# kubernetes-sigs/scheduler-plugins

Measured on AMD Instinct MI355X. Metric: pod_x_node_filter_score_evals_per_sec, higher is better.
Workload: dtype f32+f64

## Files before the change

### include/spx.h

```cpp
#ifndef SPX_H
#define SPX_H

#include <stdint.h>

#ifdef __cplusplus
extern "C" {
#endif


#define SPX_OK 0
#define SPX_ERR_ARG (-1)
#define SPX_ERR_HIP (-2)
#define SPX_ERR_STATE (-3)
#define SPX_ERR_NOGPU (-4)

#define SPX_PLUGIN_ALLOCATABLE 0
#define SPX_PLUGIN_TLP 1
#define SPX_PLUGIN_LVRB 2
#define SPX_PLUGIN_NRT 3
#define SPX_PLUGIN_NETOVERHEAD 4
#define SPX_PLUGIN_CAPACITY 5
#define SPX_PLUGIN_TOPOSORT 6
#define SPX_PLUGIN_LROC 7
#define SPX_PLUGIN_PEAKS 8
// ... 714 lines not shown
#define SPX_OPT_PEAKS_POD_CLASSES 8
#define SPX_OPT_NRT_LN_LIST_PERMILLE 9
#define SPX_OPT_COMMIT_COOP 10
#define SPX_OPT_NRT_RANK_FILTER 11
#define SPX_OPT_ROW_WORKGROUP 12
#define SPX_OPT_TLP_AMB_TABLE 13
#define SPX_OPT_NRT_PACKED_SCORE 14
#define SPX_OPT_NET_ALLOC_FUSED 15
#define SPX_OPT_NRT_RANK_NARROW 16
#define SPX_OPT_PEAKS_ESTIMATE 17
#define SPX_OPT_NRT_FUSED 18
#define SPX_OPT_NRT_WIDE 19
#define SPX_OPT_ALLOC_TABLE_KEEP 20
#define SPX_OPT_TLP_POD_CLASSES 21
#define SPX_OPT_TLP_CHUNK_SCHED 22
#define SPX_NUM_OPTIONS 23
int spx_set_option(spx_engine* e, int option, int64_t value);
int spx_get_option(const spx_engine* e, int option, int64_t* value);

int spx_nrt_pod_classes(const spx_engine* e, int64_t* n_unique, int64_t* n_copies);
int spx_peaks_pod_classes(const spx_engine* e, int64_t* n_unique, int64_t* n_copies);

int spx_tlp_pod_classes(const spx_engine* e, int64_t* rows_evaluated, int64_t* rows_copied);
int spx_tlp_form(const spx_engine* e);
int spx_tlp_fetch_order(spx_engine* e, int32_t* rows);

int spx_sysched_pod_classes(const spx_engine* e, int64_t* n_unique, int64_t* n_copies);

int spx_load_trimaran(spx_engine* e, const spx_node_objects* nodes, const spx_resource_classes* rc, const spx_pod_objects* pods, const spx_metrics_objects* metrics, const spx_assigned_objects* assigned);
int spx_load_trimaran_pods(spx_engine* e, const spx_pod_objects* pods);
int spx_load_nrt(spx_engine* e, const spx_node_objects* nodes, const spx_nrt_objects* nrt, const spx_resource_classes* rc, const spx_pod_objects* pods, const spx_nrt_params* params);
int spx_last_load_nrt_ms(const spx_engine* e, double* ms6);
int spx_load_network(spx_engine* e, const spx_node_objects* nodes, const spx_pod_objects* pods, const spx_appgroup_objects* appgroups, const spx_nettopo_objects* nettopo);
int spx_load_quota(spx_engine* e, const spx_pod_objects* pods, const spx_resource_classes* rc, const spx_quota_objects* quota);
int spx_load_sysched(spx_engine* e, const spx_sysched_objects* o);
typedef struct spx_profile_objects {
  const spx_node_objects* nodes;
  const spx_resource_classes* rc;
  const spx_pod_objects* pods;
// ... 131 lines not shown
```

### scheduler-plugins_amd/csrc/kernels_tlp_order.hip

```cpp
#include <hip/hip_runtime.h>

#include "spx_internal.h"

namespace spx {
namespace {

constexpr int kBlock = 1024;
constexpr int kSlots = 2 * kBlock;
constexpr uint32_t kEmpty = 0xffffffffu;

__device__ __forceinline__ uint32_t order_bin(int64_t v, int32_t amb_size) {
  return (v >= 0 && v < static_cast<int64_t>(amb_size)) ? static_cast<uint32_t>(v) : static_cast<uint32_t>(amb_size);
}

__device__ __forceinline__ void block_count(uint32_t* skey, uint32_t* scnt, bool live, uint32_t bin, uint32_t* slot, uint32_t* rank) {
  for (int s = threadIdx.x; s < kSlots; s += kBlock) skey[s] = kEmpty, scnt[s] = 0u;
  __syncthreads();
  *slot = 0u, *rank = 0u;
  if (live) {
    uint32_t s = (bin * 2654435761u) >> 21;
    for (;;) {
      const uint32_t prev = atomicCAS(skey + s, kEmpty, bin);
      if (prev == kEmpty || prev == bin) break;
      s = (s + 1u) & (kSlots - 1);
// ... 15 lines not shown
    if (skey[s] != kEmpty) atomicAdd(hist + skey[s], scnt[s]);
}

__device__ __forceinline__ uint32_t block_sum(uint32_t v, uint32_t* wsum) {
#pragma unroll
  for (int m = 32; m >= 1; m >>= 1) v += static_cast<uint32_t>(__shfl_xor(static_cast<int>(v), m));
  if ((threadIdx.x & 63) == 0) wsum[threadIdx.x >> 6] = v;
  __syncthreads();
  uint32_t total = 0;
#pragma unroll
  for (int w = 0; w < kBlock / 64; ++w) total += wsum[w];
  __syncthreads();
  return total;
}

__global__ __launch_bounds__(kBlock) void k_tlp_order_totals(const uint32_t* hist, int n_bins, uint32_t* totals) {
  __shared__ uint32_t wsum[kBlock / 64];
  const int b = blockIdx.x * kBlock + threadIdx.x;
  const uint32_t total = block_sum(b < n_bins ? hist[b] : 0u, wsum);
  if (threadIdx.x == 0) totals[blockIdx.x] = total;
}

__global__ __launch_bounds__(kBlock) void k_tlp_order_scan(uint32_t* hist, int n_bins, const uint32_t* totals, uint32_t* other_start, uint32_t* evaluated) {
  __shared__ uint32_t wsum[kBlock / 64];
  const int t = threadIdx.x, lane = t & 63, wave = t >> 6;
  uint32_t mine = 0;
  for (int i = t; i < static_cast<int>(blockIdx.x); i += kBlock) mine += totals[i];
  const uint32_t carry = block_sum(mine, wsum);
  const int b = blockIdx.x * kBlock + t;
  const uint32_t c = b < n_bins ? hist[b] : 0u;
  uint32_t x = c;
#pragma unroll
  for (int d = 1; d < 64; d <<= 1) {
    const uint32_t y = static_cast<uint32_t>(__shfl_up(static_cast<int>(x), d));
    if (lane >= d) x += y;
  }
  if (lane == 63) wsum[wave] = x;
  __syncthreads();
  uint32_t before = 0;
#pragma unroll
  for (int w = 0; w < kBlock / 64; ++w) before += w < wave ? wsum[w] : 0u;
  __syncthreads();
  const uint32_t o = carry + before + x - c;
  uint32_t ev = 0;
  if (b < n_bins) {
    hist[b] = o;
    if (b == n_bins - 1) *other_start = o;
    else if (c > 0u) ev = 1u + ((o + c - 1u) >> 6) - (o >> 6);
  }
  ev = block_sum(ev, wsum);
  if (t == 0 && ev != 0u) atomicAdd(evaluated, ev);
}

__global__ __launch_bounds__(kBlock) void k_tlp_order_scatter(const int64_t* pod, int64_t n, int32_t amb_size, uint32_t* cursor, int32_t* order) {
  __shared__ uint32_t skey[kSlots], scnt[kSlots];
  const int64_t r = static_cast<int64_t>(blockIdx.x) * kBlock + threadIdx.x;
  const bool live = r < n;
  uint32_t slot, rank;
  block_count(skey, scnt, live, live ? order_bin(pod[r], amb_size) : 0u, &slot, &rank);
  for (int s = threadIdx.x; s < kSlots; s += kBlock)
    if (skey[s] != kEmpty) scnt[s] = atomicAdd(cursor + skey[s], scnt[s]);
  __syncthreads();
  if (live) {
    const uint64_t pos = static_cast<uint64_t>(scnt[slot]) + rank;
    if (pos < static_cast<uint64_t>(n)) order[pos] = static_cast<int32_t>(r);
  }
}

__global__ __launch_bounds__(256) void k_tlp_order_count_key(const int64_t* pod, int64_t n, int32_t amb_size, const int32_t* order, const uint32_t* other_start,
                                                             uint32_t* evaluated, uint32_t* keys, int64_t n_chunks) {
  const int64_t p = static_cast<int64_t>(blockIdx.x) * blockDim.x + threadIdx.x;
  const uint32_t last = static_cast<uint32_t>(n - 1);
  bool ev = false, outside = false;
  if (p < n) {
    const int64_t v = pod[min(static_cast<uint32_t>(order[p]), last)];
    ev = (p & 63) == 0 || v != pod[min(static_cast<uint32_t>(order[p - 1]), last)];
    outside = order_bin(v, amb_size) == static_cast<uint32_t>(amb_size);
  }
  const unsigned long long m = __ballot(ev), mo = __ballot(ev && p >= static_cast<int64_t>(*other_start)), out = __ballot(outside);
  if ((threadIdx.x & 63) == 0) {
// ... 46 lines not shown
      for (int w = 0; w < kBlock / 64; ++w) add += wcnt[w][t], wcnt[w][t] = 0u;
      base[t] += add;
    }
    __syncthreads();
  }
}

__global__ __launch_bounds__(256) void k_tlp_order_move(int64_t n, const int32_t* sorted, const uint32_t* dest, int64_t n_chunks, int32_t* order) {
  const int64_t p = static_cast<int64_t>(blockIdx.x) * blockDim.x + threadIdx.x;
  if (p >= n) return;
  int64_t chunk = p >> 6;
  if (chunk < n_chunks) chunk = min(static_cast<int64_t>(dest[chunk]), n_chunks - 1);
  order[chunk * 64 + (p & 63)] = sorted[p];
}

}

static size_t scan_blocks(int32_t amb_size) { return (static_cast<size_t>(amb_size) + 1 + kBlock - 1) / kBlock; }
size_t tlp_order_scratch_words(int32_t amb_size, int64_t n_rows) {
  return static_cast<size_t>(amb_size) + 3 + scan_blocks(amb_size) + 2 * static_cast<size_t>(n_rows / 64) + static_cast<size_t>(n_rows);
}
size_t tlp_order_evaluated_word(int32_t amb_size) { return static_cast<size_t>(amb_size) + 2; }

void launch_tlp_order(const int64_t* pod_milli, int64_t n_rows, int32_t amb_size, bool chunk_sched, int32_t* order, uint32_t* scratch, hipStream_t s) {
  const int n_bins = amb_size + 1;
  const unsigned blocks = static_cast<unsigned>((n_rows + kBlock - 1) / kBlock), rows256 = static_cast<unsigned>((n_rows + 255) / 256);
  const unsigned sblocks = static_cast<unsigned>(scan_blocks(amb_size));
  const int64_t n_chunks = n_rows / 64;
  uint32_t* other_start = scratch + n_bins;
  uint32_t* evaluated = other_start + 1;
  uint32_t* totals = evaluated + 1;
  uint32_t* keys = totals + sblocks;
  uint32_t* dest = keys + n_chunks;
  const bool sched = chunk_sched && n_chunks > 1;
  int32_t* sorted = sched ? reinterpret_cast<int32_t*>(dest + n_chunks) : order;
  (void)hipMemsetAsync(scratch, 0, (static_cast<size_t>(n_bins) + 2) * sizeof(uint32_t), s);
  hipLaunchKernelGGL(k_tlp_order_hist, dim3(blocks), dim3(kBlock), 0, s, pod_milli, n_rows, amb_size, scratch);
  hipLaunchKernelGGL(k_tlp_order_totals, dim3(sblocks), dim3(kBlock), 0, s, scratch, n_bins, totals);
  hipLaunchKernelGGL(k_tlp_order_scan, dim3(sblocks), dim3(kBlock), 0, s, scratch, n_bins, totals, other_start, evaluated);
  hipLaunchKernelGGL(k_tlp_order_scatter, dim3(blocks), dim3(kBlock), 0, s, pod_milli, n_rows, amb_size, scratch, sorted);
  hipLaunchKernelGGL(k_tlp_order_count_key, dim3(rows256), dim3(256), 0, s, pod_milli, n_rows, amb_size, sorted, other_start, evaluated, keys, n_chunks);
  if (!sched) return;
  hipLaunchKernelGGL(k_tlp_order_sched, dim3(1), dim3(kBlock), 0, s, keys, n_chunks, dest);
  hipLaunchKernelGGL(k_tlp_order_move, dim3(rows256), dim3(256), 0, s, n_rows, sorted, dest, n_chunks, order);
}

}
```

### scheduler-plugins_amd/csrc/spx_engine.h

```cpp
#pragma once

#include <hip/hip_runtime.h>

#include <algorithm>
#include <chrono>
#include <cmath>
#include <cstdio>
#include <cstdlib>
#include <cstring>
#include <limits>
#include <string>
#include <unordered_map>
#include <vector>

#include <atomic>
#include <mutex>
#include <thread>

#include "spx_internal.h"
#include "../host/lroc_form.hpp"
#include "../host/nrt_streams.hpp"
#include "../host/parallel.hpp"

extern thread_local std::string g_create_error;
// ... 16 lines not shown
  hipStream_t own_stream = nullptr;
  hipStream_t stream = nullptr;
  hipEvent_t ev0 = nullptr, ev1 = nullptr;
  bool hold_ev0 = false;
  bool skip_alloc_masked = false;
  bool alloc_compact = false;
  bool timed = false;
  mutable std::string err;
  mutable std::mutex err_mu;
  std::mutex raw_mu;

  int64_t n_nodes = -1;
  int64_t n_pods = -1;
  int64_t row_stride = 0;

  int64_t option[SPX_NUM_OPTIONS] = {spx::kRowPad, 0, 0, 0, 0, 0, 44, 1, 1, 375, 1, 1, 0, 1, 1, 1, 1, 1, 1, 0, 1, 1, 1};

  int32_t alloc_mode = SPX_MODE_LEAST;
  std::vector<int32_t> alloc_res{SPX_RES_MEMORY, SPX_RES_CPU};
  std::vector<int64_t> alloc_weight{1, 1 << 20};
  spx_tlp_params tlp{40, 1000, 1.5};
  spx_lvrb_params lvrb{1.0, 1.0};
  int64_t plugin_weight[SPX_NUM_PLUGINS] = {1, 1, 1, 1, 1, 1, 1, 1, 1, 1};

  DevBuf d_alloc, d_alloc_w, d_alloc_raw, d_alloc_norm, d_alloc_rel;
  int32_t alloc_n_res = 0;
  bool alloc_ready = false;
  DevBuf d_alloc_prev;
  uint64_t alloc_epoch = 0;
  DevBuf d_cap_cpu, d_tlp_util, d_tlp_missing, d_tlp_valid;
  DevBuf d_lv_acpu, d_lv_amem, d_lv_cavg, d_lv_cstd, d_lv_mavg, d_lv_mstd, d_lv_flags;
  bool tri_nodes = false;
  DevBuf d_tlp_pod, d_lv_rcpu, d_lv_rmem;
  bool tri_pods = false;
  DevBuf d_raw_row;
  DevBuf d_lv_exact;
  DevBuf d_lv_fast, d_tlp_fast;
  DevBuf d_tlp_amb;
  DevBuf d_lv_amb;
  bool lv_amb_built = false;
  int64_t tlp_amb_geom[3] = {0, 0, 0}, lv_amb_geom[3] = {0, 0, 0};
  bool tlp_amb_built = false;
  DevBuf d_tlp_order, d_tlp_order_scratch;
  bool tlp_order_valid = false;
  int64_t tlp_rows_evaluated = 0;
  int tlp_last_form = 0;
  DevBuf d_commit;
  DevBuf d_decide;
  DevBuf d_stats;

  spx_lroc_params lroc{5, 0.5, 0.5};
  DevBuf d_lroc_nreq_c, d_lroc_nreq_m, d_lroc_nlim_c, d_lroc_nlim_m, d_lroc_preq_c, d_lroc_preq_m, d_lroc_plim_c, d_lroc_plim_m, d_lroc_tab, d_lroc_podf;
  bool lroc_nodes = false, lroc_pods = false, lroc_tab_ready = false;
  bool lroc_nodes_exact = false, lroc_pods_exact = false, lv_alloc_exact = false;
  bool lroc_nodes_f32 = false, lroc_pods_f32 = false, lv_alloc_f32 = false;
  int64_t lroc_node_max[4] = {0, 0, 0, 0};
  std::vector<int64_t> h_lroc_pod[4];
  bool lroc_nodes_cover = false, lroc_pods_cover = false;
  int lroc_loop_form = -1;
  bool peaks_loop_row = false;
// ... 238 lines not shown
}

int set_pods(spx_engine* e, int64_t p) {
  if (p <= 0) return fail(e, SPX_ERR_ARG, "n_pods must be positive");
  if (e->n_pods != -1 && e->n_pods != p)
    return fail(e, SPX_ERR_STATE, "n_pods differs from tables already uploaded");
  e->n_pods = p;
  return SPX_OK;
}

int tlp_build_order(spx_engine* e) {
  e->tlp_order_valid = false;
  if (e->n_pods <= 0 || e->n_pods > std::numeric_limits<int32_t>::max()) return SPX_OK;
  int rc;
  const size_t words = spx::tlp_order_scratch_words(spx::kTlpAmbSize, e->n_pods);
  if ((rc = ensure(e, e->d_tlp_order, static_cast<size_t>(e->n_pods) * sizeof(int32_t))) || (rc = ensure(e, e->d_tlp_order_scratch, words * sizeof(uint32_t))))
    return rc;
  uint32_t* scratch = static_cast<uint32_t*>(e->d_tlp_order_scratch.p);
  spx::launch_tlp_order(static_cast<const int64_t*>(e->d_tlp_pod.p), e->n_pods, spx::kTlpAmbSize, e->option[SPX_OPT_TLP_CHUNK_SCHED] != 0,
                        static_cast<int32_t*>(e->d_tlp_order.p), scratch, e->stream);
  SPX_HIP(e, hipGetLastError());
  uint32_t evaluated = 0;
  SPX_HIP(e, hipMemcpyAsync(&evaluated, scratch + spx::tlp_order_evaluated_word(spx::kTlpAmbSize), sizeof evaluated, hipMemcpyDeviceToHost, e->stream));
  SPX_HIP(e, hipStreamSynchronize(e->stream));
  e->tlp_rows_evaluated = evaluated;
  e->tlp_order_valid = true;
  return SPX_OK;
}

void alloc_table_dirty(spx_engine* e) { e->alloc_kept = spx_engine::AllocKept{}; }

int ensure_score_table(spx_engine* e, int plugin) {
  DevBuf& b = e->score[plugin];
  if (b.external) {
    if (e->score_rows[plugin] < e->n_pods || e->score_stride[plugin] < e->row_stride)
      return fail(e, SPX_ERR_STATE, "bound score table is smaller than n_pods x row_stride");
    return SPX_OK;
  }
  const size_t had = b.p ? b.bytes : 0;
  int rc = ensure(e, b, static_cast<size_t>(e->n_pods) * static_cast<size_t>(e->row_stride));
// ... 528 lines not shown
```

### scheduler-plugins_amd/csrc/spx_engine.hip

```cpp
#include "spx_engine.h"

thread_local std::string g_create_error;
thread_local std::string tl_err;
thread_local const spx_engine* tl_err_engine = nullptr;

extern "C" {

int spx_abi_version(void) { return 1; }

const char* spx_last_error(const spx_engine* e) {
  if (!e) return g_create_error.c_str();
  if (tl_err_engine != e) {
    std::lock_guard<std::mutex> g(e->err_mu);
    tl_err = e->err;
    tl_err_engine = e;
  }
  return tl_err.c_str();
}

int spx_create(int device_id, spx_engine** out) {
  if (!out) return fail(nullptr, SPX_ERR_ARG, "out is NULL");
  *out = nullptr;
  int count = 0;
  hipError_t st = hipGetDeviceCount(&count);
// ... 15 lines not shown
    delete e;
    return fail(nullptr, SPX_ERR_HIP, msg);
  }
  e->d_stats.bytes = spx::kStatBytes;
  *out = e;
  return SPX_OK;
}

int spx_destroy(spx_engine* e) {
  if (!e) return SPX_OK;
  (void)hipSetDevice(e->device);
  (void)hipStreamSynchronize(e->stream);
  DevBuf* bufs[] = {&e->d_alloc,   &e->d_alloc_w,  &e->d_alloc_raw, &e->d_alloc_norm, &e->d_alloc_rel, &e->d_alloc_prev, &e->d_cap_cpu, &e->d_tlp_util,
                    &e->d_tlp_missing, &e->d_tlp_valid, &e->d_lv_acpu, &e->d_lv_amem, &e->d_lv_cavg, &e->d_lv_cstd,
                    &e->d_lv_mavg, &e->d_lv_mstd,  &e->d_lv_flags,  &e->d_tlp_pod,    &e->d_lv_rcpu, &e->d_lv_rmem,
                    &e->d_raw_row,   &e->d_lv_exact, &e->d_lv_fast, &e->d_tlp_fast, &e->d_tlp_amb, &e->d_tlp_order, &e->d_tlp_order_scratch, &e->d_lv_amb, &e->d_nrt_pk_tab, &e->d_commit, &e->d_nrt_flags, &e->d_nrt_max_numa, &e->d_nrt_nz, &e->d_nrt_zid, &e->d_nrt_zp,
                    &e->d_nrt_avail, &e->d_nrt_cost,  &e->d_nrt_minavg, &e->d_nrt_np,    &e->d_nrt_qos, &e->d_nrt_nn,
                    &e->d_nrt_nctr,  &e->d_nrt_ckind, &e->d_nrt_cpres,  &e->d_nrt_creq,  &e->d_nrt_ppres, &e->d_nrt_preq,
                    &e->d_nrt_frcv, &e->d_nrt_fav,   &e->d_nrt_frc,   &e->d_nrt_fcpu,   &e->d_nrt_frep,  &e->d_nrt_items, &e->d_nrt_perm, &e->d_nrt_ln, &e->d_nrt_fbraw, &e->d_nrt_redo,
                    &e->d_net_region, &e->d_net_zone, &e->d_net_class, &e->d_net_class16, &e->d_net_cls_size, &e->d_net_cls_region, &e->d_net_cls_zone,
                    &e->d_net_rcost, &e->d_net_zcost, &e->d_net_pod_key, &e->d_net_key_flag, &e->d_net_pair_ptr,
                    &e->d_net_pair_node, &e->d_net_pair_max, &e->d_q_pod_ns, &e->d_q_pod_prio, &e->d_q_pod_req, &e->d_q_pod_reqp,
                    &e->d_q_has, &e->d_q_used, &e->d_q_max, &e->d_q_maxp, &e->d_q_other, &e->d_q_otherp, &e->d_q_nom_ptr,
                    &e->d_q_nom_prio, &e->d_q_nom_idx, &e->d_q_nom_req, &e->d_q_nom_reqp, &e->d_q_status, &e->d_ext_status,
                    &e->d_q_usedp, &e->d_q_min, &e->d_q_minp, &e->d_q_agg, &e->d_net_eff_ptr, &e->d_net_eff_key, &e->d_net_eff_cost, &e->d_net_dyn_ptr,
                    &e->d_net_dyn_end, &e->d_net_dyn_node, &e->d_net_dyn_max, &e->d_commit_save, &e->d_row_counter, &e->d_coop_sync, &e->d_coop_node, &e->d_coop_max,
                    &e->d_sort_prio, &e->d_sort_ts, &e->d_sort_group, &e->d_sort_topo, &e->d_sort_scratch,
                    &e->d_best, &e->d_stats, &e->d_decide, &e->d_lroc_nreq_c, &e->d_lroc_nreq_m, &e->d_lroc_nlim_c, &e->d_lroc_nlim_m,
                    &e->d_lroc_preq_c, &e->d_lroc_preq_m, &e->d_lroc_plim_c, &e->d_lroc_plim_m, &e->d_lroc_tab, &e->d_lroc_podf,
                    &e->d_pk_cap, &e->d_pk_util, &e->d_pk_valid, &e->d_pk_k1, &e->d_pk_k2, &e->d_pk_pod, &e->d_pk_min, &e->d_pk_max, &e->d_pk_rowc, &e->d_pk_tab, &e->d_pk_seg, &e->d_pk_segn,
                    &e->d_nrt_uniq, &e->d_nrt_dups, &e->d_pk_uniq, &e->d_pk_dups, &e->d_delta, &e->d_nrt_lnrec, &e->d_net_pair_node2, &e->d_net_pair_max2, &e->d_nrt_rk, &e->d_nrt_rk_off, &e->d_nrt_rk_first, &e->d_nrt_fz, &e->d_nrt_wsort, &e->d_nrt_wrank,
// ... 58 lines not shown
    case SPX_OPT_COMMIT_COOP:
    case SPX_OPT_NRT_RANK_FILTER:
    case SPX_OPT_ROW_WORKGROUP:
    case SPX_OPT_TLP_AMB_TABLE:
    case SPX_OPT_NRT_PACKED_SCORE:
    case SPX_OPT_NET_ALLOC_FUSED:
    case SPX_OPT_NRT_RANK_NARROW:
    case SPX_OPT_NRT_FUSED:
    case SPX_OPT_NRT_WIDE:
    case SPX_OPT_ALLOC_TABLE_KEEP:
    case SPX_OPT_TLP_CHUNK_SCHED:
      if (value != 0 && value != 1) return fail(e, SPX_ERR_ARG, "option takes 0 or 1");
      break;
    case SPX_OPT_TLP_POD_CLASSES:
      if (value < 0 || value > 2) return fail(e, SPX_ERR_ARG, "SPX_OPT_TLP_POD_CLASSES: 0, 1 or 2");
      break;
    case SPX_OPT_NRT_LN_LIST_PERMILLE:
      if (value < 1 || value > 1000) return fail(e, SPX_ERR_ARG, "SPX_OPT_NRT_LN_LIST_PERMILLE: 1..1000");
      break;
    case SPX_OPT_PEAKS_ESTIMATE:
      if (value != 0 && value != 1 && value != 8) return fail(e, SPX_ERR_ARG, "SPX_OPT_PEAKS_ESTIMATE: 0, 1 or 8");
      break;
    case SPX_OPT_PEAKS_TILE:
      if (value != 44 && value != 84 && value != 48 && value != 88) return fail(e, SPX_ERR_ARG, "SPX_OPT_PEAKS_TILE: 44, 84, 48 or 88");
      break;
    default:
      return fail(e, SPX_ERR_ARG, "unknown option");
  }
  e->option[option] = value;
  return SPX_OK;
// ... 523 lines not shown

int spx_nrt_filter_path(const spx_engine* e) { return e ? e->last_nrt_filter : 0; }

int spx_alloc_table_path(const spx_engine* e) { return e ? e->last_alloc_table : 0; }

int spx_tlp_pod_classes(const spx_engine* e, int64_t* rows_evaluated, int64_t* rows_copied) {
  if (!e) return SPX_ERR_ARG;
  if (!e->tri_pods || !e->tlp_order_valid) return fail(e, SPX_ERR_STATE, "TargetLoadPacking: no row order (no pod batch uploaded, or more than 2^31 - 1 rows)");
  if (rows_evaluated) *rows_evaluated = e->tlp_rows_evaluated;
  if (rows_copied) *rows_copied = e->n_pods - e->tlp_rows_evaluated;
  return SPX_OK;
}

int spx_tlp_form(const spx_engine* e) { return e ? e->tlp_last_form : 0; }

int spx_tlp_fetch_order(spx_engine* e, int32_t* rows) {
  if (!e || !rows) return SPX_ERR_ARG;
  if (!e->tri_pods || !e->tlp_order_valid) return fail(e, SPX_ERR_STATE, "TargetLoadPacking: no row order (no pod batch uploaded, or more than 2^31 - 1 rows)");
  const size_t n = static_cast<size_t>(e->n_pods);
  SPX_HIP(e, hipMemcpyAsync(rows, e->d_tlp_order.p, n * sizeof(int32_t), hipMemcpyDeviceToHost, e->stream));
  SPX_HIP(e, hipStreamSynchronize(e->stream));
  return SPX_OK;
}

int spx_nrt_wide(const spx_engine* e) { return e && e->nrt_wide ? 1 : 0; }

int spx_nrt_long_rows(const spx_engine* e, int64_t* n_out) {
  if (!e || !n_out) return SPX_ERR_ARG;
  *n_out = e->nrt_long_last;
  return SPX_OK;
// ... 435 lines not shown
  if (!(plugin_mask & C)) return decide_profile(e, plugin_mask, row_begin, row_end);
  if ((plugin_mask & ~C) == 0) return fail(e, SPX_ERR_ARG, "spx_decide: Coscheduling alone scores nothing");
  int rc;
  if ((rc = spx_eval(e, C, row_begin, row_end))) return rc;
  if ((rc = decide_profile(e, plugin_mask & ~C, row_begin, row_end))) return rc;
  const size_t P = static_cast<size_t>(e->n_pods);
  int64_t* bs = static_cast<int64_t*>(e->d_best.p);
  int32_t* bn = reinterpret_cast<int32_t*>(bs + P);
  spx::launch_cosched_unschedulable(static_cast<const uint8_t*>(e->d_cs_status.p), row_begin, row_end, bs, bn, bn + P, bn + 2 * P, e->stream);
  SPX_HIP(e, hipGetLastError());
  return SPX_OK;
}

namespace {
int decide_profile(spx_engine* e, uint32_t plugin_mask, int64_t row_begin, int64_t row_end) {
  const uint32_t A = 1u << SPX_PLUGIN_ALLOCATABLE, T = 1u << SPX_PLUGIN_TLP;
  const int kExtra[3] = {SPX_PLUGIN_LVRB, SPX_PLUGIN_LROC, SPX_PLUGIN_PEAKS};
  uint32_t extra_mask = 0;
  int64_t w_sum = 0;
  bool w_ok = true;
  for (int p = 0; p < SPX_NUM_PLUGINS; ++p)
    if (plugin_mask & (1u << p)) w_sum += e->plugin_weight[p], w_ok &= e->plugin_weight[p] >= 0;
  for (int x = 0; x < 3; ++x) extra_mask |= plugin_mask & (1u << kExtra[x]);
  const int64_t wa = e->plugin_weight[SPX_PLUGIN_ALLOCATABLE], wt = e->plugin_weight[SPX_PLUGIN_TLP];
  const bool fusable = (plugin_mask & T) && !(plugin_mask & ~(A | T | extra_mask)) && !e->ext_mask && e->tri_nodes && e->tri_pods &&
                       e->tlp.target_utilization >= 1 && e->tlp.target_utilization <= 99 && !(launch_opts(e) & spx::kOptTrimaranExact) &&
                       !e->option[SPX_OPT_DECIDE_UNFUSED] && w_ok && w_sum <= 8000;
  int rc;
  if (!fusable) {
    bool done = false;
    if ((rc = decide_masked(e, plugin_mask, plugin_mask, row_begin, row_end, &done)) || done) return rc;
  }
  if (!fusable) {
    if ((rc = spx_eval(e, plugin_mask, row_begin, row_end))) return rc;
    return spx_eval_best(e, plugin_mask, row_begin, row_end);
  }
  if (e->n_nodes <= 0 || e->n_pods <= 0) return fail(e, SPX_ERR_STATE, "shape unknown");
  if (row_begin < 0 || row_end > e->n_pods || row_begin > row_end) return fail(e, SPX_ERR_ARG, "row range out of bounds");
  const bool use_alloc = plugin_mask & A;
  if (use_alloc && (rc = prepare_alloc(e))) return rc;
  const size_t P = static_cast<size_t>(e->n_pods);
  if ((rc = ensure(e, e->d_best, P * 20))) return rc;
  if ((rc = ensure(e, e->d_tlp_fast, static_cast<size_t>(spx::round_up(e->row_stride, 1024)) * 4 * sizeof(float)))) return rc;
  if ((rc = ensure(e, e->d_decide, spx::decide_scratch_bytes(e->row_stride, row_end - row_begin)))) return rc;
  spx::DecideLaunch d{};
  fill_trimaran(e, d.t);
  d.t.row_begin = row_begin;
  d.t.row_end = row_end;
  d.t.tlp_fast = static_cast<float*>(e->d_tlp_fast.p);
  if (!e->d_tlp_amb.p) e->tlp_amb_built = false;
  if ((rc = ensure(e, e->d_tlp_amb, static_cast<size_t>(spx::kTlpAmbSize) * 4))) return rc;
  d.t.tlp_amb = static_cast<uint32_t*>(e->d_tlp_amb.p);
  d.t.tlp_amb_size = spx::kTlpAmbSize;
  d.t.tlp_amb_built = &e->tlp_amb_built;
  d.t.tlp_amb_geom = e->tlp_amb_geom;
  d.use_alloc = use_alloc;
  d.w_alloc = static_cast<int32_t>(use_alloc ? wa : 0);
  d.w_tlp = static_cast<int32_t>(wt);
  d.scratch = e->d_decide.p;
  d.best_score = static_cast<int64_t*>(e->d_best.p);
  d.best_node = reinterpret_cast<int32_t*>(d.best_score + P);
  d.best_ties = d.best_node + P;
  d.best_feasible = d.best_ties + P;
  SPX_HIP(e, hipEventRecord(e->ev0, e->stream));
  if (extra_mask) {
    e->hold_ev0 = true;
    rc = spx_eval(e, extra_mask, row_begin, row_end);
    e->hold_ev0 = false;
    if (rc) return rc;
    for (int x = 0; x < 3; ++x)
      if (extra_mask & (1u << kExtra[x])) {
        d.w_extra[d.n_extra] = static_cast<int32_t>(e->plugin_weight[kExtra[x]]);
        d.extra[d.n_extra++] = static_cast<const uint8_t*>(e->score[kExtra[x]].p);
      }
  }
  spx::launch_decide_trimaran(d, e->stream);
  SPX_HIP(e, hipGetLastError());
  SPX_HIP(e, hipEventRecord(e->ev1, e->stream));
  e->timed = true;
  e->best_valid = true;
  return SPX_OK;
}
}

extern "C" {

int spx_fetch_best(spx_engine* e, int64_t row_begin, int64_t row_end, int32_t* node_idx, int64_t* weighted_score, int32_t* n_ties,
                   int32_t* n_feasible) {
  if (!e || !node_idx || !weighted_score) return SPX_ERR_ARG;
  if (!e->best_valid) return fail(e, SPX_ERR_STATE, "spx_eval_best has not run since the last spx_eval");
  if (row_begin < 0 || row_end > e->n_pods || row_begin > row_end) return fail(e, SPX_ERR_ARG, "row range out of bounds");
  const size_t n = static_cast<size_t>(row_end - row_begin);
  const size_t P = static_cast<size_t>(e->n_pods);
  if (e->h_best_bytes < P * 20) {
    if (e->h_best) SPX_HIP(e, hipHostFree(e->h_best));
// ... 19 lines not shown
```

### scheduler-plugins_amd/csrc/spx_internal.h

```cpp
#pragma once

#include <hip/hip_runtime.h>
#include <stdint.h>

#include "../../include/spx.h"
#include "nrt_rank_layout.h"

namespace spx {

constexpr int64_t kRowAlign = 16;
constexpr int64_t kRowPad = 128;

inline int64_t round_up(int64_t v, int64_t a) { return (v + a - 1) / a * a; }

#define SPX_RESOLVE_ROWS(a)              \
  do {                                   \
    if ((a).row_ptr) {                   \
      (a).row_begin = *(a).row_ptr;      \
      (a).row_end = (a).row_begin + 1;   \
    }                                    \
  } while (0)

constexpr int kStatSlots = 64;
constexpr int kStatStride = 16;
// ... 26 lines not shown

struct AllocPrepArgs {
  int64_t n_nodes;
  int64_t row_stride;
  int32_t n_res;
  int32_t mode;
  const int64_t* alloc;
  const int64_t* weight;
  int64_t* raw;
  uint8_t* norm;
  uint32_t* rel;
};
void launch_alloc_prepare(const AllocPrepArgs& a, hipStream_t s);

constexpr int64_t kTlpClassMinCopyPct = 47;
constexpr int32_t kTlpAmbSize = 1 << 16;

struct TrimaranArgs {
  uint32_t opts;
  int64_t n_nodes;
  int64_t row_stride;
  int64_t row_begin;
  int64_t row_end;
  const int64_t* row_ptr;
  const uint8_t* alloc_norm;
  const int64_t* cap_cpu_milli;
  const double* tlp_cpu_util;
  const int64_t* tlp_missing_milli;
  const uint8_t* tlp_valid;
  const int64_t* tlp_pod_milli;
// ... 17 lines not shown
  uint32_t* lv_amb;
  int64_t* tlp_amb_geom;
  int64_t* lv_amb_geom;
  bool* lv_amb_built;
  bool* tlp_amb_built;
  const int32_t* tlp_order;
  int* tlp_form;
  unsigned long long* stats;
  uint8_t* out_alloc;
  uint8_t* out_tlp;
  uint8_t* out_lvrb;
};
void launch_trimaran(const TrimaranArgs& a, hipStream_t s);
size_t tlp_order_scratch_words(int32_t amb_size, int64_t n_rows);
size_t tlp_order_evaluated_word(int32_t amb_size);
void launch_tlp_order(const int64_t* pod_milli, int64_t n_rows, int32_t amb_size, bool chunk_sched, int32_t* order, uint32_t* scratch, hipStream_t s);
size_t lvrb_amb_bytes();
struct CommitArgs {
  TrimaranArgs t;
  uint32_t use_mask;
  int64_t w_alloc, w_tlp, w_lvrb;
  const uint8_t* lv_table;
  int64_t* missing;
  int32_t* out_node;
  int64_t* out_score;
  int32_t* out_ties;
};
void launch_commit_trimaran(const CommitArgs& c, hipStream_t s);
struct DecideLaunch {
  TrimaranArgs t;
  bool use_alloc;
// ... 750 lines not shown
```

### scheduler-plugins_amd/engine.py

```python
from __future__ import annotations

import ctypes as C
from typing import Dict, Optional, Sequence

import numpy as np

from ._abi import Table

PLUGINS = {
    "NodeResourcesAllocatable": 0,
    "TargetLoadPacking": 1,
    "LoadVariationRiskBalancing": 2,
    "NodeResourceTopologyMatch": 3,
    "NetworkOverhead": 4,
    "CapacityScheduling": 5,
    "TopologicalSort": 6,
}
ALLOCATABLE, TLP, LVRB, NRT, NETOVERHEAD, CAPACITY, TOPOSORT, LROC, PEAKS, SYSCHED = range(10)
NUM_PLUGINS = 10
COSCHED = 10
COSCHED_ST = {"BACKED_OFF": 1, "FEW_SIBLINGS": 2, "GATED": 3, "RESOURCE_GAP": 4}
PREEMPT_ST = {"CANDIDATE": 0, "NO_VICTIMS": 1, "NOT_FIT": 2, "QUOTA": 3, "ALL_REPRIEVED": 4, "REMOVE_TWICE": 5, "SKIPPED": 6}


# ... 117 lines not shown
        self._ck(self._lib.spx_peaks_pod_classes(self._h, C.byref(u), C.byref(d)))
        return int(u.value), int(d.value)

    def tlp_pod_classes(self):
        u, d = C.c_int64(), C.c_int64()
        self._ck(self._lib.spx_tlp_pod_classes(self._h, C.byref(u), C.byref(d)))
        return int(u.value), int(d.value)

    def tlp_order(self):
        rows = np.zeros(self.n_pods, np.int32)
        self._ck(self._lib.spx_tlp_fetch_order(self._h, rows.ctypes.data_as(C.POINTER(C.c_int32))))
        return rows

    def tlp_form(self) -> int:
        return int(self._lib.spx_tlp_form(self._h))

    def sysched_pod_classes(self):
        u, d = C.c_int64(), C.c_int64()
        self._ck(self._lib.spx_sysched_pod_classes(self._h, C.byref(u), C.byref(d)))
        return int(u.value), int(d.value)

    def force_reference_kernels(self, *plugins: int) -> None:
        self.set_option("REFERENCE_KERNELS", mask_of(*plugins))

    def stats(self, reset: bool = False) -> np.ndarray:
        out = np.zeros(NUM_PLUGINS, np.int64)
        self._ck(self._lib.spx_fetch_stats(self._h, out.ctypes.data_as(C.POINTER(C.c_int64)), 1 if reset else 0))
        return out

    def set_allocatable(self, mode: str = "Least", resources: Optional[Dict[int, int]] = None) -> None:
# ... 945 lines not shown
```

Measured before the change: 5720 billion.

## Deduplicate identical pods into classes for the fused decide sweep and expand results

Extends the TLP order histogram/scan/scatter kernels to assign each pod row a class id (one per distinct CPU-milli bin, with out-of-range rows kept unique) and to record a representative value per class. When the decide profile runs only Allocatable+TLP over the full batch and enough rows are duplicates, the fused decide kernel sweeps only the unique classes. A new expand kernel then copies each class result back to every row. This trades extra scan/scatter work and an expand pass for fewer pod×node evaluations, and it relies on decide results depending only on the pod's CPU-milli value in that configuration.

```diff
diff --git a/include/spx.h b/include/spx.h
--- a/include/spx.h
+++ b/include/spx.h
@@ -752,7 +752,8 @@
 #define SPX_OPT_ALLOC_TABLE_KEEP 20
 #define SPX_OPT_TLP_POD_CLASSES 21
 #define SPX_OPT_TLP_CHUNK_SCHED 22
-#define SPX_NUM_OPTIONS 23
+#define SPX_OPT_DECIDE_POD_CLASSES 23
+#define SPX_NUM_OPTIONS 24
 int spx_set_option(spx_engine* e, int option, int64_t value);
 int spx_get_option(const spx_engine* e, int option, int64_t* value);
 
@@ -761,6 +762,7 @@
 
 int spx_tlp_pod_classes(const spx_engine* e, int64_t* rows_evaluated, int64_t* rows_copied);
 int spx_tlp_form(const spx_engine* e);
+int spx_decide_pod_classes(const spx_engine* e, int64_t* rows_evaluated, int64_t* rows_copied);
 int spx_tlp_fetch_order(spx_engine* e, int32_t* rows);
 
 int spx_sysched_pod_classes(const spx_engine* e, int64_t* n_unique, int64_t* n_copies);
diff --git a/scheduler-plugins_amd/csrc/kernels_tlp_order.hip b/scheduler-plugins_amd/csrc/kernels_tlp_order.hip
--- a/scheduler-plugins_amd/csrc/kernels_tlp_order.hip
+++ b/scheduler-plugins_amd/csrc/kernels_tlp_order.hip
@@ -53,26 +53,32 @@
   return total;
 }
 
-__global__ __launch_bounds__(kBlock) void k_tlp_order_totals(const uint32_t* hist, int n_bins, uint32_t* totals) {
+__global__ __launch_bounds__(kBlock) void k_tlp_order_totals(const uint32_t* hist, int n_bins, uint32_t* totals, uint32_t* cls_totals) {
   __shared__ uint32_t wsum[kBlock / 64];
   const int b = blockIdx.x * kBlock + threadIdx.x;
-  const uint32_t total = block_sum(b < n_bins ? hist[b] : 0u, wsum);
-  if (threadIdx.x == 0) totals[blockIdx.x] = total;
-}
-
-__global__ __launch_bounds__(kBlock) void k_tlp_order_scan(uint32_t* hist, int n_bins, const uint32_t* totals, uint32_t* other_start, uint32_t* evaluated) {
+  const uint32_t c = b < n_bins ? hist[b] : 0u;
+  const uint32_t total = block_sum(c, wsum);
+  const uint32_t classes = block_sum((c > 0u && b < n_bins - 1) ? 1u : 0u, wsum);
+  if (threadIdx.x == 0) totals[blockIdx.x] = total, cls_totals[blockIdx.x] = classes;
+}
+
+__global__ __launch_bounds__(kBlock) void k_tlp_order_scan(uint32_t* hist, int n_bins, const uint32_t* totals, const uint32_t* cls_totals, uint32_t* other_start,
+                                                           uint32_t* evaluated, uint32_t* n_in_cls, uint32_t* cls_of_bin, int64_t* cls_val, int64_t n_rows) {
   __shared__ uint32_t wsum[kBlock / 64];
   const int t = threadIdx.x, lane = t & 63, wave = t >> 6;
-  uint32_t mine = 0;
-  for (int i = t; i < static_cast<int>(blockIdx.x); i += kBlock) mine += totals[i];
+  uint32_t mine = 0, mine_cls = 0;
+  for (int i = t; i < static_cast<int>(blockIdx.x); i += kBlock) mine += totals[i], mine_cls += cls_totals[i];
   const uint32_t carry = block_sum(mine, wsum);
+  const uint32_t carry_cls = block_sum(mine_cls, wsum);
   const int b = blockIdx.x * kBlock + t;
   const uint32_t c = b < n_bins ? hist[b] : 0u;
-  uint32_t x = c;
+  const uint32_t k = (c > 0u && b < n_bins - 1) ? 1u : 0u;
+  uint32_t x = c, xk = k;
 #pragma unroll
   for (int d = 1; d < 64; d <<= 1) {
     const uint32_t y = static_cast<uint32_t>(__shfl_up(static_cast<int>(x), d));
-    if (lane >= d) x += y;
+    const uint32_t yk = static_cast<uint32_t>(__shfl_up(static_cast<int>(xk), d));
+    if (lane >= d) x += y, xk += yk;
   }
   if (lane == 63) wsum[wave] = x;
   __syncthreads();
@@ -80,29 +86,51 @@
 #pragma unroll
   for (int w = 0; w < kBlock / 64; ++w) before += w < wave ? wsum[w] : 0u;
   __syncthreads();
+  if (lane == 63) wsum[wave] = xk;
+  __syncthreads();
+  uint32_t before_cls = 0;
+#pragma unroll
+  for (int w = 0; w < kBlock / 64; ++w) before_cls += w < wave ? wsum[w] : 0u;
+  __syncthreads();
   const uint32_t o = carry + before + x - c;
+  const uint32_t cls = carry_cls + before_cls + xk - k;
   uint32_t ev = 0;
   if (b < n_bins) {
     hist[b] = o;
+    cls_of_bin[b] = cls;
     if (b == n_bins - 1) *other_start = o;
-    else if (c > 0u) ev = 1u + ((o + c - 1u) >> 6) - (o >> 6);
+    else if (c > 0u) {
+      ev = 1u + ((o + c - 1u) >> 6) - (o >> 6);
+      if (static_cast<int64_t>(cls) < n_rows) cls_val[cls] = static_cast<int64_t>(b);
+    }
   }
   ev = block_sum(ev, wsum);
   if (t == 0 && ev != 0u) atomicAdd(evaluated, ev);
-}
-
-__global__ __launch_bounds__(kBlock) void k_tlp_order_scatter(const int64_t* pod, int64_t n, int32_t amb_size, uint32_t* cursor, int32_t* order) {
+  const uint32_t nk = block_sum(k, wsum);
+  if (t == 0 && nk != 0u) atomicAdd(n_in_cls, nk);
+}
+
+__global__ __launch_bounds__(kBlock) void k_tlp_order_scatter(const int64_t* pod, int64_t n, int32_t amb_size, uint32_t* cursor, int32_t* order,
+                                                              const uint32_t* other_start, const uint32_t* cls_of_bin, int64_t* cls_val, int32_t* cls_of_row) {
   __shared__ uint32_t skey[kSlots], scnt[kSlots];
   const int64_t r = static_cast<int64_t>(blockIdx.x) * kBlock + threadIdx.x;
   const bool live = r < n;
+  const int64_t v = live ? pod[r] : 0;
+  const uint32_t bin = live ? order_bin(v, amb_size) : 0u;
   uint32_t slot, rank;
-  block_count(skey, scnt, live, live ? order_bin(pod[r], amb_size) : 0u, &slot, &rank);
+  block_count(skey, scnt, live, bin, &slot, &rank);
   for (int s = threadIdx.x; s < kSlots; s += kBlock)
     if (skey[s] != kEmpty) scnt[s] = atomicAdd(cursor + skey[s], scnt[s]);
   __syncthreads();
   if (live) {
     const uint64_t pos = static_cast<uint64_t>(scnt[slot]) + rank;
     if (pos < static_cast<uint64_t>(n)) order[pos] = static_cast<int32_t>(r);
+    uint64_t cls = cls_of_bin[bin];
+    if (bin == static_cast<uint32_t>(amb_size)) {
+      cls += pos - *other_start;
+      if (cls < static_cast<uint64_t>(n)) cls_val[cls] = v;
+    }
+    cls_of_row[r] = static_cast<int32_t>(min(cls, static_cast<uint64_t>(n - 1)));
   }
 }
 
@@ -179,31 +207,55 @@
   order[chunk * 64 + (p & 63)] = sorted[p];
 }
 
+__global__ __launch_bounds__(256) void k_decide_expand(int64_t n_rows, int64_t n_cls, const int32_t* cls_of_row, const int64_t* cls_score, const int32_t* cls_node,
+                                                       const int32_t* cls_ties, const int32_t* cls_feasible, int64_t* best_score, int32_t* best_node,
+                                                       int32_t* best_ties, int32_t* best_feasible) {
+  const int64_t r = static_cast<int64_t>(blockIdx.x) * blockDim.x + threadIdx.x;
+  if (r >= n_rows) return;
+  const int64_t c = static_cast<int64_t>(min(static_cast<uint32_t>(cls_of_row[r]), static_cast<uint32_t>(n_cls - 1)));
+  best_score[r] = cls_score[c];
+  best_node[r] = cls_node[c];
+  best_ties[r] = cls_ties[c];
+  best_feasible[r] = cls_feasible[c];
+}
+
+}
+
+void launch_decide_expand(int64_t n_rows, int64_t n_cls, const int32_t* cls_of_row, const int64_t* cls_score, const int32_t* cls_node, const int32_t* cls_ties,
+                          const int32_t* cls_feasible, int64_t* best_score, int32_t* best_node, int32_t* best_ties, int32_t* best_feasible, hipStream_t s) {
+  if (n_rows <= 0 || n_cls <= 0) return;
+  hipLaunchKernelGGL(k_decide_expand, dim3(static_cast<unsigned>((n_rows + 255) / 256)), dim3(256), 0, s, n_rows, n_cls, cls_of_row, cls_score, cls_node, cls_ties,
+                     cls_feasible, best_score, best_node, best_ties, best_feasible);
 }
 
 static size_t scan_blocks(int32_t amb_size) { return (static_cast<size_t>(amb_size) + 1 + kBlock - 1) / kBlock; }
 size_t tlp_order_scratch_words(int32_t amb_size, int64_t n_rows) {
-  return static_cast<size_t>(amb_size) + 3 + scan_blocks(amb_size) + 2 * static_cast<size_t>(n_rows / 64) + static_cast<size_t>(n_rows);
+  return 2 * (static_cast<size_t>(amb_size) + 1) + 3 + 2 * scan_blocks(amb_size) + 2 * static_cast<size_t>(n_rows / 64) + static_cast<size_t>(n_rows);
 }
 size_t tlp_order_evaluated_word(int32_t amb_size) { return static_cast<size_t>(amb_size) + 2; }
 
-void launch_tlp_order(const int64_t* pod_milli, int64_t n_rows, int32_t amb_size, bool chunk_sched, int32_t* order, uint32_t* scratch, hipStream_t s) {
+void launch_tlp_order(const int64_t* pod_milli, int64_t n_rows, int32_t amb_size, bool chunk_sched, int32_t* order, uint32_t* scratch, int64_t* cls_val,
+                      int32_t* cls_of_row, hipStream_t s) {
   const int n_bins = amb_size + 1;
   const unsigned blocks = static_cast<unsigned>((n_rows + kBlock - 1) / kBlock), rows256 = static_cast<unsigned>((n_rows + 255) / 256);
   const unsigned sblocks = static_cast<unsigned>(scan_blocks(amb_size));
   const int64_t n_chunks = n_rows / 64;
   uint32_t* other_start = scratch + n_bins;
   uint32_t* evaluated = other_start + 1;
-  uint32_t* totals = evaluated + 1;
-  uint32_t* keys = totals + sblocks;
+  uint32_t* n_in_cls = evaluated + 1;
+  uint32_t* totals = n_in_cls + 1;
+  uint32_t* cls_totals = totals + sblocks;
+  uint32_t* keys = cls_totals + sblocks;
   uint32_t* dest = keys + n_chunks;
+  uint32_t* cls_of_bin = dest + n_chunks + n_rows;
   const bool sched = chunk_sched && n_chunks > 1;
   int32_t* sorted = sched ? reinterpret_cast<int32_t*>(dest + n_chunks) : order;
-  (void)hipMemsetAsync(scratch, 0, (static_cast<size_t>(n_bins) + 2) * sizeof(uint32_t), s);
+  (void)hipMemsetAsync(scratch, 0, (static_cast<size_t>(n_bins) + 3) * sizeof(uint32_t), s);
   hipLaunchKernelGGL(k_tlp_order_hist, dim3(blocks), dim3(kBlock), 0, s, pod_milli, n_rows, amb_size, scratch);
-  hipLaunchKernelGGL(k_tlp_order_totals, dim3(sblocks), dim3(kBlock), 0, s, scratch, n_bins, totals);
-  hipLaunchKernelGGL(k_tlp_order_scan, dim3(sblocks), dim3(kBlock), 0, s, scratch, n_bins, totals, other_start, evaluated);
-  hipLaunchKernelGGL(k_tlp_order_scatter, dim3(blocks), dim3(kBlock), 0, s, pod_milli, n_rows, amb_size, scratch, sorted);
+  hipLaunchKernelGGL(k_tlp_order_totals, dim3(sblocks), dim3(kBlock), 0, s, scratch, n_bins, totals, cls_totals);
+  hipLaunchKernelGGL(k_tlp_order_scan, dim3(sblocks), dim3(kBlock), 0, s, scratch, n_bins, totals, cls_totals, other_start, evaluated, n_in_cls, cls_of_bin, cls_val,
+                     n_rows);
+  hipLaunchKernelGGL(k_tlp_order_scatter, dim3(blocks), dim3(kBlock), 0, s, pod_milli, n_rows, amb_size, scratch, sorted, other_start, cls_of_bin, cls_val, cls_of_row);
   hipLaunchKernelGGL(k_tlp_order_count_key, dim3(rows256), dim3(256), 0, s, pod_milli, n_rows, amb_size, sorted, other_start, evaluated, keys, n_chunks);
   if (!sched) return;
   hipLaunchKernelGGL(k_tlp_order_sched, dim3(1), dim3(kBlock), 0, s, keys, n_chunks, dest);
diff --git a/scheduler-plugins_amd/csrc/spx_engine.h b/scheduler-plugins_amd/csrc/spx_engine.h
--- a/scheduler-plugins_amd/csrc/spx_engine.h
+++ b/scheduler-plugins_amd/csrc/spx_engine.h
@@ -54,7 +54,7 @@
   int64_t n_pods = -1;
   int64_t row_stride = 0;
 
-  int64_t option[SPX_NUM_OPTIONS] = {spx::kRowPad, 0, 0, 0, 0, 0, 44, 1, 1, 375, 1, 1, 0, 1, 1, 1, 1, 1, 1, 0, 1, 1, 1};
+  int64_t option[SPX_NUM_OPTIONS] = {spx::kRowPad, 0, 0, 0, 0, 0, 44, 1, 1, 375, 1, 1, 0, 1, 1, 1, 1, 1, 1, 0, 1, 1, 1, 1};
 
   int32_t alloc_mode = SPX_MODE_LEAST;
   std::vector<int32_t> alloc_res{SPX_RES_MEMORY, SPX_RES_CPU};
@@ -84,6 +84,10 @@
   DevBuf d_tlp_order, d_tlp_order_scratch;
   bool tlp_order_valid = false;
   int64_t tlp_rows_evaluated = 0;
+  DevBuf d_tlp_cls_val, d_tlp_cls_of_row, d_best_cls;
+  int64_t tlp_n_cls = 0;
+  int decide_last_form = 0;
+  int64_t decide_last_rows = 0;
   int tlp_last_form = 0;
   DevBuf d_commit;
   DevBuf d_decide;
@@ -352,16 +356,20 @@
   if (e->n_pods <= 0 || e->n_pods > std::numeric_limits<int32_t>::max()) return SPX_OK;
   int rc;
   const size_t words = spx::tlp_order_scratch_words(spx::kTlpAmbSize, e->n_pods);
-  if ((rc = ensure(e, e->d_tlp_order, static_cast<size_t>(e->n_pods) * sizeof(int32_t))) || (rc = ensure(e, e->d_tlp_order_scratch, words * sizeof(uint32_t))))
+  if ((rc = ensure(e, e->d_tlp_order, static_cast<size_t>(e->n_pods) * sizeof(int32_t))) || (rc = ensure(e, e->d_tlp_order_scratch, words * sizeof(uint32_t))) ||
+      (rc = ensure(e, e->d_tlp_cls_val, static_cast<size_t>(e->n_pods) * sizeof(int64_t))) ||
+      (rc = ensure(e, e->d_tlp_cls_of_row, static_cast<size_t>(e->n_pods) * sizeof(int32_t))))
     return rc;
   uint32_t* scratch = static_cast<uint32_t*>(e->d_tlp_order_scratch.p);
   spx::launch_tlp_order(static_cast<const int64_t*>(e->d_tlp_pod.p), e->n_pods, spx::kTlpAmbSize, e->option[SPX_OPT_TLP_CHUNK_SCHED] != 0,
-                        static_cast<int32_t*>(e->d_tlp_order.p), scratch, e->stream);
+                        static_cast<int32_t*>(e->d_tlp_order.p), scratch, static_cast<int64_t*>(e->d_tlp_cls_val.p),
+                        static_cast<int32_t*>(e->d_tlp_cls_of_row.p), e->stream);
   SPX_HIP(e, hipGetLastError());
-  uint32_t evaluated = 0;
-  SPX_HIP(e, hipMemcpyAsync(&evaluated, scratch + spx::tlp_order_evaluated_word(spx::kTlpAmbSize), sizeof evaluated, hipMemcpyDeviceToHost, e->stream));
+  uint32_t words3[3] = {0, 0, 0};
+  SPX_HIP(e, hipMemcpyAsync(words3, scratch + spx::tlp_order_evaluated_word(spx::kTlpAmbSize) - 1, sizeof words3, hipMemcpyDeviceToHost, e->stream));
   SPX_HIP(e, hipStreamSynchronize(e->stream));
-  e->tlp_rows_evaluated = evaluated;
+  e->tlp_rows_evaluated = words3[1];
+  e->tlp_n_cls = std::min<int64_t>(e->n_pods, static_cast<int64_t>(words3[2]) + std::max<int64_t>(0, e->n_pods - static_cast<int64_t>(words3[0])));
   e->tlp_order_valid = true;
   return SPX_OK;
 }
diff --git a/scheduler-plugins_amd/csrc/spx_engine.hip b/scheduler-plugins_amd/csrc/spx_engine.hip
--- a/scheduler-plugins_amd/csrc/spx_engine.hip
+++ b/scheduler-plugins_amd/csrc/spx_engine.hip
@@ -53,7 +53,7 @@
   DevBuf* bufs[] = {&e->d_alloc,   &e->d_alloc_w,  &e->d_alloc_raw, &e->d_alloc_norm, &e->d_alloc_rel, &e->d_alloc_prev, &e->d_cap_cpu, &e->d_tlp_util,
                     &e->d_tlp_missing, &e->d_tlp_valid, &e->d_lv_acpu, &e->d_lv_amem, &e->d_lv_cavg, &e->d_lv_cstd,
                     &e->d_lv_mavg, &e->d_lv_mstd,  &e->d_lv_flags,  &e->d_tlp_pod,    &e->d_lv_rcpu, &e->d_lv_rmem,
-                    &e->d_raw_row,   &e->d_lv_exact, &e->d_lv_fast, &e->d_tlp_fast, &e->d_tlp_amb, &e->d_tlp_order, &e->d_tlp_order_scratch, &e->d_lv_amb, &e->d_nrt_pk_tab, &e->d_commit, &e->d_nrt_flags, &e->d_nrt_max_numa, &e->d_nrt_nz, &e->d_nrt_zid, &e->d_nrt_zp,
+                    &e->d_raw_row,   &e->d_lv_exact, &e->d_lv_fast, &e->d_tlp_fast, &e->d_tlp_amb, &e->d_tlp_order, &e->d_tlp_order_scratch, &e->d_tlp_cls_val, &e->d_tlp_cls_of_row, &e->d_best_cls, &e->d_lv_amb, &e->d_nrt_pk_tab, &e->d_commit, &e->d_nrt_flags, &e->d_nrt_max_numa, &e->d_nrt_nz, &e->d_nrt_zid, &e->d_nrt_zp,
                     &e->d_nrt_avail, &e->d_nrt_cost,  &e->d_nrt_minavg, &e->d_nrt_np,    &e->d_nrt_qos, &e->d_nrt_nn,
                     &e->d_nrt_nctr,  &e->d_nrt_ckind, &e->d_nrt_cpres,  &e->d_nrt_creq,  &e->d_nrt_ppres, &e->d_nrt_preq,
                     &e->d_nrt_frcv, &e->d_nrt_fav,   &e->d_nrt_frc,   &e->d_nrt_fcpu,   &e->d_nrt_frep,  &e->d_nrt_items, &e->d_nrt_perm, &e->d_nrt_ln, &e->d_nrt_fbraw, &e->d_nrt_redo,
@@ -142,6 +142,9 @@
       break;
     case SPX_OPT_TLP_POD_CLASSES:
       if (value < 0 || value > 2) return fail(e, SPX_ERR_ARG, "SPX_OPT_TLP_POD_CLASSES: 0, 1 or 2");
+      break;
+    case SPX_OPT_DECIDE_POD_CLASSES:
+      if (value < 0 || value > 2) return fail(e, SPX_ERR_ARG, "SPX_OPT_DECIDE_POD_CLASSES: 0, 1 or 2");
       break;
     case SPX_OPT_NRT_LN_LIST_PERMILLE:
       if (value < 1 || value > 1000) return fail(e, SPX_ERR_ARG, "SPX_OPT_NRT_LN_LIST_PERMILLE: 1..1000");
@@ -695,6 +698,14 @@
 
 int spx_tlp_form(const spx_engine* e) { return e ? e->tlp_last_form : 0; }
 
+int spx_decide_pod_classes(const spx_engine* e, int64_t* rows_evaluated, int64_t* rows_copied) {
+  if (!e) return 0;
+  const bool fused = e->decide_last_form != 0;
+  if (rows_evaluated) *rows_evaluated = fused ? e->decide_last_rows : 0;
+  if (rows_copied) *rows_copied = e->decide_last_form == 2 ? e->n_pods - e->decide_last_rows : 0;
+  return e->decide_last_form;
+}
+
 int spx_tlp_fetch_order(spx_engine* e, int32_t* rows) {
   if (!e || !rows) return SPX_ERR_ARG;
   if (!e->tri_pods || !e->tlp_order_valid) return fail(e, SPX_ERR_STATE, "TargetLoadPacking: no row order (no pod batch uploaded, or more than 2^31 - 1 rows)");
@@ -1160,6 +1171,8 @@
 
 namespace {
 int decide_profile(spx_engine* e, uint32_t plugin_mask, int64_t row_begin, int64_t row_end) {
+  e->decide_last_form = 0;
+  e->decide_last_rows = 0;
   const uint32_t A = 1u << SPX_PLUGIN_ALLOCATABLE, T = 1u << SPX_PLUGIN_TLP;
   const int kExtra[3] = {SPX_PLUGIN_LVRB, SPX_PLUGIN_LROC, SPX_PLUGIN_PEAKS};
   uint32_t extra_mask = 0;
@@ -1188,11 +1201,21 @@
   const size_t P = static_cast<size_t>(e->n_pods);
   if ((rc = ensure(e, e->d_best, P * 20))) return rc;
   if ((rc = ensure(e, e->d_tlp_fast, static_cast<size_t>(spx::round_up(e->row_stride, 1024)) * 4 * sizeof(float)))) return rc;
-  if ((rc = ensure(e, e->d_decide, spx::decide_scratch_bytes(e->row_stride, row_end - row_begin)))) return rc;
+  bool cls = false;
+  const int64_t cls_opt = e->option[SPX_OPT_DECIDE_POD_CLASSES];
+  if (cls_opt && !extra_mask && e->tlp_order_valid && row_begin == 0 && row_end == e->n_pods && !e->row_indirect && e->tlp_n_cls > 0 && e->tlp_n_cls < e->n_pods) {
+    const int64_t copied = e->n_pods - e->tlp_n_cls;
+    cls = cls_opt == 2 || copied * 100 >= spx::kDecideClassMinCopyPct * e->n_pods;
+  }
+  const int64_t sweep_rows = cls ? e->tlp_n_cls : row_end - row_begin;
+  if ((rc = ensure(e, e->d_decide, spx::decide_scratch_bytes(e->row_stride, sweep_rows)))) return rc;
+  if (cls && (rc = ensure(e, e->d_best_cls, static_cast<size_t>(sweep_rows) * 20))) return rc;
   spx::DecideLaunch d{};
   fill_trimaran(e, d.t);
-  d.t.row_begin = row_begin;
-  d.t.row_end = row_end;
+  d.t.row_begin = cls ? 0 : row_begin;
+  d.t.row_end = cls ? sweep_rows : row_end;
+  d.t.tlp_order = nullptr;
+  if (cls) d.t.tlp_pod_milli = static_cast<const int64_t*>(e->d_tlp_cls_val.p);
   d.t.tlp_fast = static_cast<float*>(e->d_tlp_fast.p);
   if (!e->d_tlp_amb.p) e->tlp_amb_built = false;
   if ((rc = ensure(e, e->d_tlp_amb, static_cast<size_t>(spx::kTlpAmbSize) * 4))) return rc;
@@ -1204,10 +1227,11 @@
   d.w_alloc = static_cast<int32_t>(use_alloc ? wa : 0);
   d.w_tlp = static_cast<int32_t>(wt);
   d.scratch = e->d_decide.p;
-  d.best_score = static_cast<int64_t*>(e->d_best.p);
-  d.best_node = reinterpret_cast<int32_t*>(d.best_score + P);
-  d.best_ties = d.best_node + P;
-  d.best_feasible = d.best_ties + P;
+  const size_t BP = cls ? static_cast<size_t>(sweep_rows) : P;
+  d.best_score = static_cast<int64_t*>(cls ? e->d_best_cls.p : e->d_best.p);
+  d.best_node = reinterpret_cast<int32_t*>(d.best_score + BP);
+  d.best_ties = d.best_node + BP;
+  d.best_feasible = d.best_ties + BP;
   SPX_HIP(e, hipEventRecord(e->ev0, e->stream));
   if (extra_mask) {
     e->hold_ev0 = true;
@@ -1221,10 +1245,18 @@
       }
   }
   spx::launch_decide_trimaran(d, e->stream);
+  if (cls) {
+    int64_t* bs = static_cast<int64_t*>(e->d_best.p);
+    int32_t* bn = reinterpret_cast<int32_t*>(bs + P);
+    spx::launch_decide_expand(e->n_pods, sweep_rows, static_cast<const int32_t*>(e->d_tlp_cls_of_row.p), d.best_score, d.best_node, d.best_ties, d.best_feasible, bs,
+                              bn, bn + P, bn + 2 * P, e->stream);
+  }
   SPX_HIP(e, hipGetLastError());
   SPX_HIP(e, hipEventRecord(e->ev1, e->stream));
   e->timed = true;
   e->best_valid = true;
+  e->decide_last_form = cls ? 2 : 1;
+  e->decide_last_rows = sweep_rows;
   return SPX_OK;
 }
 }
diff --git a/scheduler-plugins_amd/csrc/spx_internal.h b/scheduler-plugins_amd/csrc/spx_internal.h
--- a/scheduler-plugins_amd/csrc/spx_internal.h
+++ b/scheduler-plugins_amd/csrc/spx_internal.h
@@ -64,6 +64,7 @@
 void launch_alloc_prepare(const AllocPrepArgs& a, hipStream_t s);
 
 constexpr int64_t kTlpClassMinCopyPct = 47;
+constexpr int64_t kDecideClassMinCopyPct = 12;
 constexpr int32_t kTlpAmbSize = 1 << 16;
 
 struct TrimaranArgs {
@@ -111,7 +112,10 @@
 void launch_trimaran(const TrimaranArgs& a, hipStream_t s);
 size_t tlp_order_scratch_words(int32_t amb_size, int64_t n_rows);
 size_t tlp_order_evaluated_word(int32_t amb_size);
-void launch_tlp_order(const int64_t* pod_milli, int64_t n_rows, int32_t amb_size, bool chunk_sched, int32_t* order, uint32_t* scratch, hipStream_t s);
+void launch_tlp_order(const int64_t* pod_milli, int64_t n_rows, int32_t amb_size, bool chunk_sched, int32_t* order, uint32_t* scratch, int64_t* cls_val,
+                      int32_t* cls_of_row, hipStream_t s);
+void launch_decide_expand(int64_t n_rows, int64_t n_cls, const int32_t* cls_of_row, const int64_t* cls_score, const int32_t* cls_node, const int32_t* cls_ties,
+                          const int32_t* cls_feasible, int64_t* best_score, int32_t* best_node, int32_t* best_ties, int32_t* best_feasible, hipStream_t s);
 size_t lvrb_amb_bytes();
 struct CommitArgs {
   TrimaranArgs t;
diff --git a/scheduler-plugins_amd/engine.py b/scheduler-plugins_amd/engine.py
--- a/scheduler-plugins_amd/engine.py
+++ b/scheduler-plugins_amd/engine.py
@@ -155,6 +155,11 @@
 
     def tlp_form(self) -> int:
         return int(self._lib.spx_tlp_form(self._h))
+
+    def decide_pod_classes(self):
+        u, d = C.c_int64(), C.c_int64()
+        form = int(self._lib.spx_decide_pod_classes(self._h, C.byref(u), C.byref(d)))
+        return form, int(u.value), int(d.value)
 
     def sysched_pod_classes(self):
         u, d = C.c_int64(), C.c_int64()
```

Result: slower. 4758 billion (-16.8%).
